# jondeaton/PhaMers

Hardware: AMD Instinct MI355X
Metric: Gbases/s k-mer-count+score, k=4, 5 kb contigs (higher is better)
Workload: dtype u32 counts + f16 MFMA proposal (exact integer counts x fp16 reference parts, f32 accumulate; k=4: high parts in the sweep, low parts added in f64 to the window's candidates) + f64 decision; 1 GPU; BASELINE configs[1]: k=4, 1000000 x 5000-base contigs per GPU, count+normalise+combo score, 4510 reference rows + 172 centroids; contigs_per_gpu=1000000, contig_length=5000, k=4, method=combo, parallelism=contig shards, 1 rank(s), replicated reference, final all-gather of scores

## Files before the change

### phamers_amd/csrc/phk_common.h

```cpp
#pragma once
#include <hip/hip_runtime.h>
#include <stdint.h>
#include <stdarg.h>
#include <stdio.h>
#include <string>
#include <thread>
#include <functional>
#include <vector>

#include "../../include/phamers_hip.h"

#define PHK_WAVE 64

#if (defined(I8_TIMERS) || defined(I8_NW) || defined(I8_NBUF) || defined(PHK_HI_REFINE) || \
     defined(PHK_RERANK_WAVES) || defined(PAIRS_ABL) || defined(F16H_ABL)) && !defined(PHK_DIAGNOSTIC_BUILD)
#error "kernel tuning / timer macros need -DPHK_DIAGNOSTIC_BUILD (make EXTRA_CXXFLAGS='-DPHK_DIAGNOSTIC_BUILD -D...')"
#endif

void phk_set_error(const char *fmt, ...);

#define PHK_HIP(call)                                                                      \
    do {                                                                                   \
        hipError_t e__ = (call);                                                           \
        if (e__ != hipSuccess) {                                                           \
            phk_set_error("%s failed: %s (%s:%d)", #call, hipGetErrorString(e__), __FILE__, \
                          __LINE__);                                                       \
            return e__ == hipErrorOutOfMemory ? PHK_ERR_NOMEM : PHK_ERR_HIP;               \
        }                                                                                  \
    } while (0)

#define PHK_REQUIRE(cond, ...)        \
    do {                              \
        if (!(cond)) {                \
            phk_set_error(__VA_ARGS__); \
            return PHK_ERR_ARG;       \
        }                             \
    } while (0)

#define PHK_ENTER(ctx_, fname)                                   \
    do {                                                         \
        PHK_REQUIRE((ctx_) != nullptr, fname ": NULL ctx");      \
        PHK_HIP(hipSetDevice((ctx_)->device));                   \
    } while (0)

#define PHK_TRY(call)               \
    do {                            \
        int rc__ = (call);          \
        if (rc__ != PHK_OK) return rc__; \
    } while (0)

enum PhkSlot {
    WS_ASCII = 0,
    WS_PACKED,
    WS_MASK,
    WS_OFFSETS,
    WS_COUNTS,
    WS_WIDE,
    WS_FLAGS,
    WS_Q64,
    WS_SCORES,
    WS_DIST,
    WS_QF32,
    WS_CAND,
    WS_NWIN,
    WS_LONG,
    WS_OUT,
    WS_SUB,
    WS_QUEUE,
    WS_FRAG8,
    WS_BIG8,
    WS_SCTL,
    WS_CTL,
    WS_KDE,
    WS_SORT,
    WS_NN,
    WS_NNF,
    WS_NND,
    WS_SLOTS
};

struct PhkBuf {
    void *ptr = nullptr;
    uint64_t bytes = 0;
    uint64_t gen = 0;
};

struct PhkTimed {
    std::string name;
    std::vector<hipEvent_t> ev;
    double ms = 0.0;
    uint64_t launches = 0;
};

struct PhkLayout {
    uint64_t bytes = 0;
    uint64_t align = 256;
    uint64_t take(uint64_t b) {
        const uint64_t o = bytes;
        bytes += (b + align - 1) / align * align;
        return o;
    }
};

enum PhkProposal { PHK_PROP_DEFAULT = 0, PHK_PROP_OTHER, PHK_PROP_F16, PHK_PROP_HI, PHK_PROP_CXF, PHK_PROP_I83 };

struct PhkKnobs {
    char count_lanes = 0;
    bool force_exact = false;
    PhkProposal proposal = PHK_PROP_DEFAULT;
    char cx_cfg[8] = "";
    char rerank = 0;
    bool count_sort = true;
    uint64_t score_batch = 0;
    char i8_insert = 0;
    bool gen_seq = false;
    int gen_groups = 0;
    int ws_fail = 0;
    bool tail_aside = true;
};

#define PHK_PREP8_MISSING 0x40000000u
#define PHK_I8_L1_MAX 65000u
struct PhkPrep8 {
    bool offered = false;
    bool written = false;
    const uint32_t *counts = nullptr;
    uint64_t n = 0, D = 0;
    void *frag = nullptr;
    uint32_t *big = nullptr;
};

struct PhkStepLink {
    PhkPrep8 prep8;
    uint32_t *zero[2] = {nullptr, nullptr};
    uint32_t zero_words[2] = {0, 0};
    bool planned = false;
    bool zeroed(const uint32_t *p) const { return planned && p && (p == zero[0] || p == zero[1]); }
};

struct phk_ctx {
    int device = 0;
    PhkKnobs knobs;
    bool slots_lds0 = true;
    hipStream_t stream = nullptr;
    bool own_stream = false;
    hipStream_t aux = nullptr;
    hipEvent_t ev_fork[2] = {nullptr, nullptr}, ev_tail[2] = {nullptr, nullptr};
    uint64_t ctl_gen = 0, ctl_epoch = 0;
    bool ctl_dirty = true;
    uint64_t score_ctl_gen = 0;
    bool score_ctl_dirty = true;
    int num_cus = 256;
    PhkBuf ws[WS_SLOTS];
    bool profile = false;
    bool last_score_fast = false;
    std::vector<PhkTimed> timed;
    std::vector<hipEvent_t> ev_pool;
    void *stage[2] = {nullptr, nullptr};
    uint64_t stage_bytes = 0;
    uint64_t nn_queries = 0, nn_fell_back = 0;
    bool nn_keep = false;
    uint64_t nn_det_n = 0;
    int nn_det_k = 0;
};

int phk_ws(phk_ctx *ctx, int slot, uint64_t bytes, void **out);

struct phk_batch {
// ... 112 lines not shown
```

### phamers_amd/csrc/score_decide.hip

```cpp
#include "score_decide.h"

template <int SRC>
__global__ __launch_bounds__(256) void phk_decide_kernel(const void *__restrict__ src, RerankParams p) {
    __shared__ uint32_t s_ix[2][256];
    __shared__ double s_T[256], s_nq2[256], s_nqp2[256], s_dp2[256], s_dn2[256], s_opQ[256], s_opI[256], s_opH[256];
    const int tid = threadIdx.x, lane = tid & 63, t = lane & 15;
    const int QB = blockDim.x;
    const uint64_t qb = (uint64_t)blockIdx.x * QB;
    const bool want_knn = (p.method & PHK_METHOD_KNN) != 0, want_cen = (p.method & PHK_METHOD_KMEANS) != 0;

    auto rowptr = [&](int pass) {
        const int ql = pass * (QB / 16) + (tid >> 4);
        const uint64_t q = qb + ql < p.N ? qb + ql : p.N - 1;
        return reinterpret_cast<const uint2 *>(static_cast<const uint32_t *>(src) + q * FAST_D) + t;
    };
    uint2 pre[2][8];
    if (SRC == 0) {
#pragma unroll
        for (int i = 0; i < 8; ++i) {
            pre[0][i] = rowptr(0)[16 * i];
            pre[1][i] = rowptr(1)[16 * i];
        }
    }

// ... 230 lines not shown
                const bool up = x > v[k];
                const float tv = v[k];
                const uint32_t ti = ix[k];
                v[k] = up ? x : tv;
                ix[k] = up ? xi : ti;
                x = up ? tv : x;
                xi = up ? ti : xi;
            }
        }
        gap_hi[sg] = need == 1 ? v[0] : need == 2 ? v[1] : v[2];
        gap_lo[sg] = need == 1 ? v[1] : need == 2 ? v[2] : v[3];
        filled[sg] = (need == 1 ? ix[0] : need == 2 ? ix[1] : ix[2]) < ncols;
#pragma unroll
        for (int r = 0; r < 3; ++r) lead[sg][r] = ix[r];
    }
    s_ix[0][tid] = lead[1][0] < (uint32_t)p.n_cpos ? lead[1][0] : 0u;
    s_ix[1][tid] = lead[2][0] < (uint32_t)p.n_cneg ? lead[2][0] : 0u;
    {
        uint32_t fl = 0;
#pragma unroll
        for (int sg = 0; sg < NSEG; ++sg) {
            s_gap[sg][0][tid] = gap_hi[sg];
            s_gap[sg][1][tid] = gap_lo[sg];
            s_gap[sg][2][tid] = Useg[sg];
            fl |= filled[sg] ? 1u << sg : 0u;
        }
#pragma unroll
        for (int r = 0; r < 3; ++r) fl |= p.labels[lead[0][r] < (uint32_t)p.M ? lead[0][r] : 0u] ? 16u << r : 0u;
        s_flag[tid] = fl;
    }
    __syncthreads();

#pragma unroll 1
    for (int pass = 0; pass < 16; ++pass) {
        const int ql = pass * 4 + grp;
        const uint64_t q = qb + ql < p.N ? qb + ql : p.N - 1;
        const double Tq = (double)p.rowsum[q];
        const uint4 *row = reinterpret_cast<const uint4 *>(counts + q * D) + t;
        const double *cp = p.C64 + (uint64_t)s_ix[0][ql] * D, *cn = p.C64 + (p.n_cpos + (uint64_t)s_ix[1][ql]) * D;
        double ssq = 0.0, ap = 0.0, dp[4] = {0.0, 0.0, 0.0, 0.0}, dn[4] = {0.0, 0.0, 0.0, 0.0};
#pragma unroll 1
        for (int ch = 0; ch < NCH; ++ch) {
#pragma unroll 1
            for (int io = 0; io < LPC / 4; ++io) {
            uint4 c[4];
#pragma unroll
            for (int i = 0; i < 4; ++i) c[i] = row[ch * (CHUNK / 4) + 16 * (4 * io + i)];
#pragma unroll
            for (int i = 0; i < 4; ++i) {
                const int d0 = ch * CHUNK + 64 * (4 * io + i) + 4 * t;
                const double x[4] = {(double)c[i].x, (double)c[i].y, (double)c[i].z, (double)c[i].w};
                const double2 m0 = *reinterpret_cast<const double2 *>(s_mu + d0), m1 = *reinterpret_cast<const double2 *>(s_mu + d0 + 2);
                const double mu4[4] = {m0.x, m0.y, m1.x, m1.y};
                double2 a0 = {0.0, 0.0}, a1 = {0.0, 0.0}, b0 = {0.0, 0.0}, b1 = {0.0, 0.0};
                if (want_cen) {
                    a0 = *reinterpret_cast<const double2 *>(cp + d0); a1 = *reinterpret_cast<const double2 *>(cp + d0 + 2);
                    b0 = *reinterpret_cast<const double2 *>(cn + d0); b1 = *reinterpret_cast<const double2 *>(cn + d0 + 2);
                }
                const double ca[4] = {a0.x, a0.y, a1.x, a1.y}, cb[4] = {b0.x, b0.y, b1.x, b1.y};
#pragma unroll
                for (int e = 0; e < 4; ++e) {
                    ssq = fma(x[e], x[e], ssq);
                    const double qm = fma(-Tq, mu4[e], x[e]);
                    ap = fma(qm, qm, ap);
                }
                if (want_cen) {
                    const double e0 = fma(-Tq, ca[0], x[0]), e1 = fma(-Tq, ca[1], x[1]), e2 = fma(-Tq, ca[2], x[2]), e3 = fma(-Tq, ca[3], x[3]);
                    dp[i & 3] = fma(e0, e0, fma(e1, e1, fma(e2, e2, fma(e3, e3, dp[i & 3]))));
                    const double f0 = fma(-Tq, cb[0], x[0]), f1 = fma(-Tq, cb[1], x[1]), f2 = fma(-Tq, cb[2], x[2]), f3 = fma(-Tq, cb[3], x[3]);
                    dn[i & 3] = fma(f0, f0, fma(f1, f1, fma(f2, f2, fma(f3, f3, dn[i & 3]))));
                }
            }
            }
        }
        ssq = group16_sum(ssq);
        ap = group16_sum(ap);
        double dps = 0.0, dns = 0.0;
        if (want_cen) {
            dps = (group16_sum(dp[0]) + group16_sum(dp[1])) + (group16_sum(dp[2]) + group16_sum(dp[3]));
            dns = (group16_sum(dn[0]) + group16_sum(dn[1])) + (group16_sum(dn[2]) + group16_sum(dn[3]));
        }
        if (t == 0) {
            s_ssq[ql] = ssq;
            s_nqp2[ql] = ap;
            s_dp2[ql] = dps;
            s_dn2[ql] = dns;
        }
    }
    __syncthreads();

    bool slow = false;
    if (in_a) {
        const uint32_t Tu = p.rowsum[qa];
        const uint32_t fl = s_flag[tid];
        if (Tu == 0u) {
            p.scores[p.q_base + qa] = __builtin_nan("");
            if (p.status) atomicAdd(p.status, 1u);
        } else {
            const double Tq = (double)Tu, ry = 1.0 / Tq, invT2 = 1.0 / (Tq * Tq);
            const double ssq = s_ssq[tid], nqp2 = s_nqp2[tid] * invT2;
            const double vs = p.vscale * ry;
            const double rcen = (double)phk_row_center(Tu, D);
            const CenteredOperand cop = phk_centered_operand_fast(ssq, Tq, ry, rcen, rcen, (double)D, p.eb_hsum);
            ErrBound eb;
            eb.A = phk_sqrt_up(ssq * (ry * ry) * (1.0 + 1e-12)) + p.mu_norm;
            eb.P = phk_sqrt_up(nqp2 + cop.shift2);
            eb.Q = cop.Q; eb.I = cop.I; eb.habs = cop.habs;
            eb.cA = p.eb_cA; eb.cP = p.eb_cP; eb.cR = p.eb_cR; eb.cabs = p.eb_abs; eb.cQ = p.eb_cQ; eb.cI = p.eb_cI; eb.cIf = p.eb_cIf;
            const double eps_g = eb(p.rmax);
            auto as_it_stands = [&](int sg) {
                if (!((fl >> sg) & 1u)) return false;
                const double el = cop.Q * p.lam8[sg] * (1.0 + 1.0e-6);
                const double thr = (double)s_gap[sg][0][tid] * vs - 2.0 * (el + eps_g);
                return (double)s_gap[sg][2][tid] * vs < thr && (double)s_gap[sg][1][tid] * vs < thr;
            };
            bool ok = true;
            double knn = 0.0;
            if (want_knn) {
                ok = as_it_stands(0);
                int votes = 0;
                for (int r = 0; r < p.kn; ++r) votes += (fl >> (4 + r)) & 1u;
                knn = (2 * votes > p.kn) ? 1.0 : -1.0;
            }
            if (want_cen) ok = ok && as_it_stands(1) && as_it_stands(2);
            if (ok) {
                if (want_cen) {
                    const uint64_t oq = p.out_map ? (uint64_t)p.out_map[qa] : qa;
                    if (p.pend) {
                        p.pend[2 * oq] = s_dp2[tid] * invT2;
                        p.pend[2 * oq + 1] = s_dn2[tid] * invT2;
                        p.scores[p.q_base + oq] = knn;
                    } else {
                        const double ep = sqrt(s_dp2[tid] * invT2), en = sqrt(s_dn2[tid] * invT2);
                        p.scores[p.q_base + oq] = knn + tanh((en - ep) / (ep + en));
                    }
                } else {
                    p.scores[p.q_base + (p.out_map ? (uint64_t)p.out_map[qa] : qa)] = knn;
                }
            } else {
                slow = true;
            }
        }
    }
    const unsigned long long sm = __ballot(slow);
    if (sm) {
        uint32_t base = 0;
        if (tid == 0) base = atomicAdd(p.fb_count + 2, (uint32_t)__popcll(sm));
        base = __shfl(base, 0);
        if (slow) p.slow_list[base + (uint32_t)__popcll(sm & ((1ull << tid) - 1ull))] = (uint32_t)qa;
    }
}

template <bool KNN, bool CEN>
__global__ __launch_bounds__(64) void phk_decide_h_kernel(const uint32_t *__restrict__ counts, RerankParams p, HiParams hp) {
    __shared__ uint32_t s_c0[8][64];
    __shared__ uint32_t s_ix[2][64];
    __shared__ float s_corr[PHK_HI_REFINE][64];
    __shared__ float s_v8[8][64], s_u0[64], s_ch[4][64];
    __shared__ double s_cn[5][64];
    __shared__ uint32_t s_flags[64];
    __shared__ double s_T[64], s_sumsq[64], s_apsum[64], s_dp2[64], s_dn2[64];
    __shared__ uint32_t s_cmx[64], s_cmn[64];
    __shared__ double s_mu[FAST_D];
    const int tid = threadIdx.x, t = tid & 15;
    const uint64_t qb = (uint64_t)blockIdx.x * 64;
    constexpr bool want_knn = KNN, want_cen = CEN;
    auto rowptr = [&](int pass) {
        const int ql = pass * 4 + (tid >> 4);
        const uint64_t q = qb + ql < p.N ? qb + ql : p.N - 1;
        return reinterpret_cast<const uint2 *>(counts + q * FAST_D) + t;
    };
    uint2 cur[8];
#pragma unroll
    for (int i = 0; i < 8; ++i) cur[i] = rowptr(0)[16 * i];
    {
        const double2 m2a = reinterpret_cast<const double2 *>(p.mu64)[2 * tid], m2b = reinterpret_cast<const double2 *>(p.mu64)[2 * tid + 1];
        reinterpret_cast<double2 *>(s_mu)[2 * tid] = m2a;
        reinterpret_cast<double2 *>(s_mu)[2 * tid + 1] = m2b;
    }

    const uint64_t qa = qb + tid;
    const bool in_a = qa < p.N;
    const uint64_t qc = in_a ? qa : p.N - 1;
    float v8[8];
    uint32_t i8[8];
    float U0 = 0.f;
    bool ok0 = true;
    float ch1[2] = {0.f, 0.f}, ch2[2] = {0.f, 0.f};
    uint32_t cl[2] = {0u, 0u};
    bool cfill[2] = {true, true};
    {
        float lv[NSEG][8], lu[2] = {0.f, 0.f};
        uint32_t li[NSEG][8];
        if (KNN) {
            lu[0] = p.cand_u[candu_at(0, 0, qc, p.N)];
            lu[1] = p.cand_u[candu_at(0, 1, qc, p.N)];
        }
#pragma unroll
        for (int sg = 0; sg < NSEG; ++sg)
            if (sg == 0 ? KNN : CEN) {
#pragma unroll
                for (int c = 0; c < 8; ++c) {
                    li[sg][c] = p.cand_i[cand_at(sg, c >> 2, c & 3, qc, p.N)];
                    lv[sg][c] = p.cand_v[cand_at(sg, c >> 2, c & 3, qc, p.N)];
                }
            }
        __builtin_amdgcn_sched_barrier(0);
        if (KNN) {
            U0 = fmaxf(lu[0], lu[1]);
#pragma unroll
            for (int c = 0; c < 8; ++c) {
                v8[c] = li[0][c] >= (uint32_t)p.M ? -3.0e38f : lv[0][c];
                i8[c] = li[0][c];
            }
#pragma unroll
            for (int a = 1; a < 8; ++a)
#pragma unroll
                for (int b = a; b > 0; --b) {
                    const bool sw = v8[b] > v8[b - 1];
                    const float tv = v8[b]; const uint32_t ti = i8[b];
                    v8[b] = sw ? v8[b - 1] : v8[b]; i8[b] = sw ? i8[b - 1] : i8[b];
                    v8[b - 1] = sw ? tv : v8[b - 1]; i8[b - 1] = sw ? ti : i8[b - 1];
                }
        }
        if (CEN) {
#pragma unroll
            for (int sg = 1; sg <= 2; ++sg) {
                const uint32_t ncols = sg == 1 ? (uint32_t)p.n_cpos : (uint32_t)p.n_cneg;
                float b1 = -3.0e38f, b2 = -3.0e38f;
                uint32_t bi = 0xFFFFFFFFu;
#pragma unroll
                for (int c = 0; c < 8; ++c) {
                    const uint32_t ix = li[sg][c];
                    const float w = ix >= ncols ? -3.0e38f : lv[sg][c];
                    const bool up = w > b1;
                    b2 = up ? b1 : fmaxf(b2, w);
                    bi = up ? ix : bi;
                    b1 = up ? w : b1;
                }
                ch1[sg - 1] = b1; ch2[sg - 1] = b2; cl[sg - 1] = bi;
                cfill[sg - 1] = bi < ncols;
            }
        }
    }
    const uint32_t ixp = cl[0] < (uint32_t)p.n_cpos ? cl[0] : 0u, ixn = cl[1] < (uint32_t)p.n_cneg ? cl[1] : 0u;
    s_ix[0][tid] = ixp;
    s_ix[1][tid] = ixn;
    {
        double cn0[3];
        uint8_t lab[8];
        uint32_t c8[8];
#pragma unroll
        for (int r = 0; r < 8; ++r) c8[r] = (KNN && i8[r] < (uint32_t)p.M) ? i8[r] : 0u;
#pragma unroll
        for (int r = 0; r < 8; ++r) {
            if (r < 3) cn0[r] = p.colnorm[c8[r]];
            lab[r] = p.labels[c8[r]];
        }
        const double cnp = p.colnorm[p.M + ixp], cnn = p.colnorm[p.M + p.n_cpos + ixn];
        __builtin_amdgcn_sched_barrier(0);
        uint32_t labbits = 0;
#pragma unroll
        for (int r = 0; r < 8; ++r) {
            labbits |= (uint32_t)(lab[r] ? 1u : 0u) << r;
            s_c0[r][tid] = c8[r];
            s_v8[r][tid] = (KNN && i8[r] < (uint32_t)p.M) ? v8[r] : -3.0e38f;
        }
        if (KNN) ok0 = i8[p.kn - 1] < (uint32_t)p.M;
        s_u0[tid] = U0;
        s_ch[0][tid] = ch1[0]; s_ch[1][tid] = ch2[0]; s_ch[2][tid] = ch1[1]; s_ch[3][tid] = ch2[1];
        s_cn[0][tid] = cn0[0]; s_cn[1][tid] = cn0[1]; s_cn[2][tid] = cn0[2]; s_cn[3][tid] = cnp; s_cn[4][tid] = cnn;
        s_flags[tid] = labbits | (ok0 ? 0x100u : 0u) | (cfill[0] ? 0x200u : 0u) | (cfill[1] ? 0x400u : 0u);
    }
    __syncthreads();

#pragma unroll 2
    for (int pass = 0; pass < 16; ++pass) {
        const int ql = pass * 4 + (tid >> 4);
        double2 ca[8], cb[8];
        uint4 l0[PHK_HI_REFINE], l1[PHK_HI_REFINE];
        uint2 nxt[8];
        if (CEN) {
            const double2 *ra = reinterpret_cast<const double2 *>(p.C64 + (uint64_t)s_ix[0][ql] * FAST_D) + t;
            const double2 *rb = reinterpret_cast<const double2 *>(p.C64 + (p.n_cpos + (uint64_t)s_ix[1][ql]) * FAST_D) + t;
#pragma unroll
            for (int i = 0; i < 8; ++i) {
                ca[i] = ra[16 * i];
                cb[i] = rb[16 * i];
            }
        }
        if (KNN) {
#pragma unroll
            for (int r = 0; r < PHK_HI_REFINE; ++r) {
                const uint4 *lp = reinterpret_cast<const uint4 *>(hp.lo16 + (uint64_t)s_c0[r][ql] * FAST_D) + t;
                l0[r] = lp[0];
                l1[r] = lp[16];
            }
        }
        {
            const uint2 *nrow = rowptr((pass + 1) & 15);
#pragma unroll
            for (int i = 0; i < 8; ++i) nxt[i] = nrow[16 * i];
        }
        __builtin_amdgcn_sched_barrier(0);
        double qd[16];
        uint32_t sum = 0, cmx = 0, cmn = 0xFFFFFFFFu;
#pragma unroll
        for (int i = 0; i < 8; ++i) {
            const uint2 c = cur[i];
            sum += c.x + c.y;
            cmx = max(cmx, max(c.x, c.y));
            cmn = min(cmn, min(c.x, c.y));
            qd[2 * i + 0] = (double)c.x;
            qd[2 * i + 1] = (double)c.y;
        }
        sum = group16_sum(sum);
        cmx = group16_max(cmx);
        cmn = group16_min(cmn);
        const bool bad = sum == 0;
        const double Tq = (double)sum;
        double dp2 = 0.0, dn2 = 0.0;
        if (CEN) {
            double acca = 0.0, accb = 0.0;
#pragma unroll
            for (int i = 0; i < 8; ++i) {
                const double a0 = fma(-Tq, ca[i].x, qd[2 * i]), a1 = fma(-Tq, ca[i].y, qd[2 * i + 1]);
                const double b0 = fma(-Tq, cb[i].x, qd[2 * i]), b1 = fma(-Tq, cb[i].y, qd[2 * i + 1]);
                acca = fma(a0, a0, fma(a1, a1, acca));
                accb = fma(b0, b0, fma(b1, b1, accb));
            }
            dp2 = group16_sum(acca);
            dn2 = group16_sum(accb);
        }
        double aq = 0.0, ap = 0.0;
#pragma unroll
        for (int i = 0; i < 8; ++i) {
            const double2 m2 = reinterpret_cast<const double2 *>(s_mu)[16 * i + t];
            aq = fma(qd[2 * i], qd[2 * i], fma(qd[2 * i + 1], qd[2 * i + 1], aq));
            qd[2 * i] = fma(-Tq, m2.x, qd[2 * i]);
            qd[2 * i + 1] = fma(-Tq, m2.y, qd[2 * i + 1]);
            ap = fma(qd[2 * i], qd[2 * i], fma(qd[2 * i + 1], qd[2 * i + 1], ap));
        }
        const double sumsq = group16_sum(aq), apsum = group16_sum(ap);
        if (KNN) {
            const double dlt = (double)phk_row_center(sum, FAST_D) - Tq * (1.0 / FAST_D);
            float qf[16];
#pragma unroll
            for (int i = 0; i < 16; ++i) qf[i] = (float)(qd[i] - dlt);
#pragma unroll
            for (int r = 0; r < PHK_HI_REFINE; ++r) {
                const _Float16 *lh0 = reinterpret_cast<const _Float16 *>(&l0[r]), *lh1 = reinterpret_cast<const _Float16 *>(&l1[r]);
                float acc = 0.f;
#pragma unroll
                for (int i = 0; i < 8; ++i) {
                    acc = fmaf(qf[i], (float)lh0[i], acc);
                    acc = fmaf(qf[8 + i], (float)lh1[i], acc);
                }
                acc = group16_sum(acc);
                if (t == 0) s_corr[r][ql] = acc;
            }
        }
        if (t == 0) {
            s_T[ql] = bad ? 0.0 : Tq;
            s_sumsq[ql] = sumsq;
            s_apsum[ql] = apsum;
            s_dp2[ql] = dp2;
            s_dn2[ql] = dn2;
            s_cmx[ql] = cmx;
            s_cmn[ql] = cmn;
        }
#pragma unroll
        for (int i = 0; i < 8; ++i) cur[i] = nxt[i];
    }
    __syncthreads();

    if (!in_a) return;
    const double Tq = s_T[tid];
    if (Tq == 0.0) {
        p.scores[p.q_base + qa] = __builtin_nan("");
        if (p.status) atomicAdd(p.status, 1u);
        return;
    }
    const double invT2 = 1.0 / (Tq * Tq);
    const double nq2 = s_sumsq[tid] * invT2, nqp2 = s_apsum[tid] * invT2;
    const CenteredOperand cop = phk_centered_operand(s_sumsq[tid], Tq, (double)s_cmx[tid], (double)s_cmn[tid], (double)FAST_D, p.eb_hsum);
    const double vs = p.vscale / Tq;
    double cn0[3];
    uint32_t labbits;
    {
#pragma unroll
        for (int r = 0; r < 8; ++r) v8[r] = s_v8[r][tid];
        U0 = s_u0[tid];
        ch1[0] = s_ch[0][tid]; ch2[0] = s_ch[1][tid]; ch1[1] = s_ch[2][tid]; ch2[1] = s_ch[3][tid];
        cn0[0] = s_cn[0][tid]; cn0[1] = s_cn[1][tid]; cn0[2] = s_cn[2][tid];
        const uint32_t fl = s_flags[tid];
        labbits = fl & 0xFFu;
        ok0 = (fl & 0x100u) != 0;
        cfill[0] = (fl & 0x200u) != 0;
        cfill[1] = (fl & 0x400u) != 0;
    }
    const double cnp2 = s_cn[3][tid], cnn2 = s_cn[4][tid];
    ErrBound eb;
    eb.A = sqrt(nq2) + p.mu_norm;
    eb.P = sqrt(nqp2);
    eb.Q = cop.Q; eb.I = cop.I; eb.habs = cop.habs + p.eb_babs;
    eb.cA = p.eb_cA; eb.cP = p.eb_cP; eb.cR = p.eb_cR; eb.cabs = p.eb_abs; eb.cQ = p.eb_cQ; eb.cI = p.eb_cI; eb.cIf = p.eb_cIf;
    eb.cM = p.eb_cM; eb.M = p.eb_M;
    const double nqp = eb.P;
    const double nqx = sqrt(nqp2 + cop.shift2);
    auto e_hi = [&](int sg, double R) { return nqx * phk_lam_of(hp, sg, R) + eb(R); };
    bool cert = true;
    bool cert_c = true;
    double knn = 0.0, cen = 0.0;
    if (want_knn) {
        const int need = p.kn;
        cert = ok0;
        if (cert) {
            const double eg = e_hi(0, p.rmax);
            const double d2up = fmax(nqp2 - 2.0 * ((double)v8[need - 1] * vs - eg), 0.0);
            const double R0 = fmin(p.rmax, (nqp + sqrt(d2up)) * (1.0 + 1e-6));
            bool near = true;
            for (int r = 0; r < need; ++r) near = near && cn0[r] <= R0;
            const double Rw = near ? R0 : p.rmax;
            const double eh = near ? e_hi(0, R0) : eg, e22 = eb(Rw) + 0x1p-19 * nqx * phk_lam_of(hp, 0, Rw);
            const double thr = (double)v8[need - 1] * vs - 2.0 * eh;
            int nw = 0;
#pragma unroll
            for (int r = 0; r < 8; ++r) nw += ((double)v8[r] * vs >= thr && v8[r] > -1.0e38f) ? 1 : 0;
            cert = nw <= PHK_HI_REFINE && (double)U0 * vs < thr;
            if (!cert && nw > PHK_HI_REFINE) atomicAdd(phk_stat_word(p, p.counters + 8, 8), 1u);
            if (!cert && nw <= PHK_HI_REFINE) atomicAdd(phk_stat_word(p, p.counters + 9, 9), 1u);
            if (cert) {
                double rv[PHK_HI_REFINE];
                uint32_t rl[PHK_HI_REFINE];
#pragma unroll
                for (int r = 0; r < PHK_HI_REFINE; ++r) {
                    const bool in = r < nw;
                    rv[r] = in ? ((double)v8[r] + (double)s_corr[r][tid]) * vs : -1.0e300;
                    rl[r] = (labbits >> r) & 1u;
                }
#pragma unroll
                for (int a = 1; a < PHK_HI_REFINE; ++a)
#pragma unroll
                    for (int b = a; b > 0; --b) {
                        const bool sw = rv[b] > rv[b - 1];
                        const double tv = rv[b]; const uint32_t tl = rl[b];
                        rv[b] = sw ? rv[b - 1] : rv[b]; rl[b] = sw ? rl[b - 1] : rl[b];
                        rv[b - 1] = sw ? tv : rv[b - 1]; rl[b - 1] = sw ? tl : rl[b - 1];
                    }
                const double hi_v = need == 1 ? rv[0] : need == 2 ? rv[1] : rv[2];
                const double lo_v = need == 1 ? rv[1] : need == 2 ? rv[2] : rv[3];
                cert = nw == need || hi_v - lo_v > 2.0 * e22;
                if (!cert) atomicAdd(phk_stat_word(p, p.counters + 10, 10), 1u);
                int votes = 0;
                for (int r = 0; r < need; ++r) votes += (int)rl[r];
                knn = (2 * votes > need) ? 1.0 : -1.0;
            }
        }
    }
    if (want_cen) {
        auto leader_ok = [&](int k2, double cnorm) {
            if (!cfill[k2]) return false;
            const double eg = e_hi(1 + k2, p.rmax);
            const double d2up = fmax(nqp2 - 2.0 * ((double)ch1[k2] * vs - eg), 0.0);
            const double R0 = fmin(p.rmax, (nqp + sqrt(d2up)) * (1.0 + 1e-6));
            const double eh = cnorm <= R0 ? e_hi(1 + k2, R0) : eg;
            return ((double)ch1[k2] - (double)ch2[k2]) * vs > 2.0 * eh;
        };
        cert_c = leader_ok(0, cnp2) && leader_ok(1, cnn2);
        if (!cert_c) atomicAdd(phk_stat_word(p, p.counters + 11, 11), 1u);
        const double ep = sqrt(s_dp2[tid] * invT2), en = sqrt(s_dn2[tid] * invT2);
        cen = tanh((en - ep) / (ep + en));
    }
    if (cert && cert_c) {
        p.scores[p.q_base + qa] = knn + cen;
    } else {
        p.scores[p.q_base + qa] = (cert ? knn : 0.0) + (cert_c ? cen : 0.0);
        const uint32_t open_parts = ((want_knn && !cert) ? 1u : 0u) | ((want_cen && !cert_c) ? 2u : 0u);
        if (p.sub_lists) {
            const uint32_t sl = blockIdx.x % p.sub_lists;
            uint32_t *cw = p.stripes + sl * 32u;
            const uint64_t base = (uint64_t)sl * p.sub_cap;
            if (open_parts == 2u) p.slow_list[base + p.sub_cap - 1 - atomicAdd(cw + 12, 1u)] = (uint32_t)qa | (open_parts << 30);
            else p.slow_list[base + atomicAdd(cw + 2, 1u)] = (uint32_t)qa | (open_parts << 30);
        } else if (open_parts == 2u) p.slow_list[p.slow_cap - 1 - atomicAdd(p.counters + 12, 1u)] = (uint32_t)qa | (open_parts << 30);
        else p.slow_list[atomicAdd(p.fb_count + 2, 1u)] = (uint32_t)qa | (open_parts << 30);
    }
}

int phk_launch_decide(phk_ctx *ctx, int src_kind, const void *src, const RerankParams &p) {
    const dim3 grid((unsigned)phk_div_up(p.N, 64));
    if (src_kind == 0) { PHK_LAUNCH(ctx, "phk_decide_kernel", phk_decide_kernel<0><<<grid, dim3(64), 0, ctx->stream>>>(src, p)); }
    else { PHK_LAUNCH(ctx, "phk_decide_kernel", phk_decide_kernel<1><<<grid, dim3(64), 0, ctx->stream>>>(src, p)); }
    return PHK_OK;
}

int phk_launch_decide_gen(phk_ctx *ctx, int dsub, const uint32_t *counts, const RerankParams &p) {
    const dim3 grid((unsigned)phk_div_up(p.N, 64));
#define PHK_DG(DS) PHK_LAUNCH(ctx, "phk_decide_gen_kernel", (phk_decide_gen_kernel<DS><<<grid, dim3(64), 0, ctx->stream>>>(counts, p)))
    switch (dsub) {
        case 2: PHK_DG(2); break;
        case 4: PHK_DG(4); break;
        case 8: PHK_DG(8); break;
        case 16: PHK_DG(16); break;
        default: phk_set_error("phk_launch_decide_gen: D = %d", 256 * dsub); return PHK_ERR_UNSUPPORTED;
    }
#undef PHK_DG
    return PHK_OK;
}

int phk_launch_decide_h(phk_ctx *ctx, bool knn, bool cen, dim3 grid, dim3 block, const uint32_t *counts, const RerankParams &p, const HiParams &hp) {
    PHK_REQUIRE(knn || cen, "phk_launch_decide_h: nothing to decide");
    if (knn && cen) { PHK_LAUNCH(ctx, "phk_decide_h_kernel", (phk_decide_h_kernel<true, true><<<grid, block, 0, ctx->stream>>>(counts, p, hp))); }
    else if (knn) { PHK_LAUNCH(ctx, "phk_decide_h_kernel", (phk_decide_h_kernel<true, false><<<grid, block, 0, ctx->stream>>>(counts, p, hp))); }
    else { PHK_LAUNCH(ctx, "phk_decide_h_kernel", (phk_decide_h_kernel<false, true><<<grid, block, 0, ctx->stream>>>(counts, p, hp))); }
    return PHK_OK;
}
```

Before: 1473 Gbases/s.

## Compact fp16 low-part refinement to only queries whose window has ties

The decide kernel used to load the low fp16 reference parts for every query's top candidates and compute correction dot products during the main 16-pass sweep. Now the certification bounds are evaluated first, the queries that actually need refinement (certified with more window candidates than k) are compacted into a shared list, and only those rows are reloaded and corrected in a second, wave-compacted loop. The change also keeps mu in registers instead of shared memory, shares LDS between the row sums and the correction buffer through a union, and adds an occupancy hint to the launch bounds. In exchange, refined rows are read twice, extra barriers are added, and register pressure under the new launch bound may cause spills.

```diff
diff --git a/phamers_amd/csrc/phk_common.h b/phamers_amd/csrc/phk_common.h
--- a/phamers_amd/csrc/phk_common.h
+++ b/phamers_amd/csrc/phk_common.h
@@ -13,7 +13,8 @@
 #define PHK_WAVE 64
 
 #if (defined(I8_TIMERS) || defined(I8_NW) || defined(I8_NBUF) || defined(PHK_HI_REFINE) || \
-     defined(PHK_RERANK_WAVES) || defined(PAIRS_ABL) || defined(F16H_ABL)) && !defined(PHK_DIAGNOSTIC_BUILD)
+     defined(PHK_RERANK_WAVES) || defined(PAIRS_ABL) || defined(F16H_ABL) || defined(PHK_DECIDE_H_CLASSES)) && \
+    !defined(PHK_DIAGNOSTIC_BUILD)
 #error "kernel tuning / timer macros need -DPHK_DIAGNOSTIC_BUILD (make EXTRA_CXXFLAGS='-DPHK_DIAGNOSTIC_BUILD -D...')"
 #endif
 
diff --git a/phamers_amd/csrc/score_decide.hip b/phamers_amd/csrc/score_decide.hip
--- a/phamers_amd/csrc/score_decide.hip
+++ b/phamers_amd/csrc/score_decide.hip
@@ -406,32 +406,27 @@
 }
 
 template <bool KNN, bool CEN>
-__global__ __launch_bounds__(64) void phk_decide_h_kernel(const uint32_t *__restrict__ counts, RerankParams p, HiParams hp) {
-    __shared__ uint32_t s_c0[8][64];
+__global__ __launch_bounds__(64, 3) void phk_decide_h_kernel(const uint32_t *__restrict__ counts, RerankParams p, HiParams hp) {
+    __shared__ uint32_t s_c0[PHK_HI_REFINE][64];
     __shared__ uint32_t s_ix[2][64];
-    __shared__ float s_corr[PHK_HI_REFINE][64];
     __shared__ float s_v8[8][64], s_u0[64], s_ch[4][64];
     __shared__ double s_cn[5][64];
     __shared__ uint32_t s_flags[64];
-    __shared__ double s_T[64], s_sumsq[64], s_apsum[64], s_dp2[64], s_dn2[64];
-    __shared__ uint32_t s_cmx[64], s_cmn[64];
-    __shared__ double s_mu[FAST_D];
+    __shared__ double s_T[64], s_dp2[64], s_dn2[64];
+    struct RowSums { double sumsq[64], apsum[64]; uint32_t cmx[64], cmn[64]; };
+    __shared__ union { RowSums row; float corr[PHK_HI_REFINE][64]; } s_w;
+    __shared__ uint8_t s_list[64];
     const int tid = threadIdx.x, t = tid & 15;
     const uint64_t qb = (uint64_t)blockIdx.x * 64;
     constexpr bool want_knn = KNN, want_cen = CEN;
-    auto rowptr = [&](int pass) {
-        const int ql = pass * 4 + (tid >> 4);
+    auto rowptr_of = [&](int ql) {
         const uint64_t q = qb + ql < p.N ? qb + ql : p.N - 1;
         return reinterpret_cast<const uint2 *>(counts + q * FAST_D) + t;
     };
+    auto rowptr = [&](int pass) { return rowptr_of(pass * 4 + (tid >> 4)); };
     uint2 cur[8];
 #pragma unroll
     for (int i = 0; i < 8; ++i) cur[i] = rowptr(0)[16 * i];
-    {
-        const double2 m2a = reinterpret_cast<const double2 *>(p.mu64)[2 * tid], m2b = reinterpret_cast<const double2 *>(p.mu64)[2 * tid + 1];
-        reinterpret_cast<double2 *>(s_mu)[2 * tid] = m2a;
-        reinterpret_cast<double2 *>(s_mu)[2 * tid + 1] = m2b;
-    }
 
     const uint64_t qa = qb + tid;
     const bool in_a = qa < p.N;
@@ -517,7 +512,7 @@
 #pragma unroll
         for (int r = 0; r < 8; ++r) {
             labbits |= (uint32_t)(lab[r] ? 1u : 0u) << r;
-            s_c0[r][tid] = c8[r];
+            if (r < PHK_HI_REFINE) s_c0[r][tid] = c8[r];
             s_v8[r][tid] = (KNN && i8[r] < (uint32_t)p.M) ? v8[r] : -3.0e38f;
         }
         if (KNN) ok0 = i8[p.kn - 1] < (uint32_t)p.M;
@@ -528,11 +523,14 @@
     }
     __syncthreads();
 
+    double2 mu[8];
+#pragma unroll
+    for (int i = 0; i < 8; ++i) mu[i] = reinterpret_cast<const double2 *>(p.mu64)[16 * i + t];
+
 #pragma unroll 2
     for (int pass = 0; pass < 16; ++pass) {
         const int ql = pass * 4 + (tid >> 4);
         double2 ca[8], cb[8];
-        uint4 l0[PHK_HI_REFINE], l1[PHK_HI_REFINE];
         uint2 nxt[8];
         if (CEN) {
             const double2 *ra = reinterpret_cast<const double2 *>(p.C64 + (uint64_t)s_ix[0][ql] * FAST_D) + t;
@@ -543,21 +541,12 @@
                 cb[i] = rb[16 * i];
             }
         }
-        if (KNN) {
-#pragma unroll
-            for (int r = 0; r < PHK_HI_REFINE; ++r) {
-                const uint4 *lp = reinterpret_cast<const uint4 *>(hp.lo16 + (uint64_t)s_c0[r][ql] * FAST_D) + t;
-                l0[r] = lp[0];
-                l1[r] = lp[16];
-            }
-        }
         {
             const uint2 *nrow = rowptr((pass + 1) & 15);
 #pragma unroll
             for (int i = 0; i < 8; ++i) nxt[i] = nrow[16 * i];
         }
         __builtin_amdgcn_sched_barrier(0);
-        double qd[16];
         uint32_t sum = 0, cmx = 0, cmn = 0xFFFFFFFFu;
 #pragma unroll
         for (int i = 0; i < 8; ++i) {
@@ -565,164 +554,211 @@
             sum += c.x + c.y;
             cmx = max(cmx, max(c.x, c.y));
             cmn = min(cmn, min(c.x, c.y));
-            qd[2 * i + 0] = (double)c.x;
-            qd[2 * i + 1] = (double)c.y;
         }
         sum = group16_sum(sum);
         cmx = group16_max(cmx);
         cmn = group16_min(cmn);
         const bool bad = sum == 0;
         const double Tq = (double)sum;
+        double aq = 0.0, ap = 0.0, acca = 0.0, accb = 0.0;
+#pragma unroll
+        for (int i = 0; i < 8; ++i) {
+            const double x0 = (double)cur[i].x, x1 = (double)cur[i].y;
+            if (CEN) {
+                const double a0 = fma(-Tq, ca[i].x, x0), a1 = fma(-Tq, ca[i].y, x1);
+                const double b0 = fma(-Tq, cb[i].x, x0), b1 = fma(-Tq, cb[i].y, x1);
+                acca = fma(a0, a0, fma(a1, a1, acca));
+                accb = fma(b0, b0, fma(b1, b1, accb));
+            }
+            aq = fma(x0, x0, fma(x1, x1, aq));
+            const double y0 = fma(-Tq, mu[i].x, x0), y1 = fma(-Tq, mu[i].y, x1);
+            ap = fma(y0, y0, fma(y1, y1, ap));
+        }
         double dp2 = 0.0, dn2 = 0.0;
         if (CEN) {
-            double acca = 0.0, accb = 0.0;
-#pragma unroll
-            for (int i = 0; i < 8; ++i) {
-                const double a0 = fma(-Tq, ca[i].x, qd[2 * i]), a1 = fma(-Tq, ca[i].y, qd[2 * i + 1]);
-                const double b0 = fma(-Tq, cb[i].x, qd[2 * i]), b1 = fma(-Tq, cb[i].y, qd[2 * i + 1]);
-                acca = fma(a0, a0, fma(a1, a1, acca));
-                accb = fma(b0, b0, fma(b1, b1, accb));
-            }
             dp2 = group16_sum(acca);
             dn2 = group16_sum(accb);
         }
-        double aq = 0.0, ap = 0.0;
-#pragma unroll
-        for (int i = 0; i < 8; ++i) {
-            const double2 m2 = reinterpret_cast<const double2 *>(s_mu)[16 * i + t];
-            aq = fma(qd[2 * i], qd[2 * i], fma(qd[2 * i + 1], qd[2 * i + 1], aq));
-            qd[2 * i] = fma(-Tq, m2.x, qd[2 * i]);
-            qd[2 * i + 1] = fma(-Tq, m2.y, qd[2 * i + 1]);
-            ap = fma(qd[2 * i], qd[2 * i], fma(qd[2 * i + 1], qd[2 * i + 1], ap));
-        }
         const double sumsq = group16_sum(aq), apsum = group16_sum(ap);
-        if (KNN) {
-            const double dlt = (double)phk_row_center(sum, FAST_D) - Tq * (1.0 / FAST_D);
-            float qf[16];
-#pragma unroll
-            for (int i = 0; i < 16; ++i) qf[i] = (float)(qd[i] - dlt);
-#pragma unroll
-            for (int r = 0; r < PHK_HI_REFINE; ++r) {
-                const _Float16 *lh0 = reinterpret_cast<const _Float16 *>(&l0[r]), *lh1 = reinterpret_cast<const _Float16 *>(&l1[r]);
-                float acc = 0.f;
-#pragma unroll
-                for (int i = 0; i < 8; ++i) {
-                    acc = fmaf(qf[i], (float)lh0[i], acc);
-                    acc = fmaf(qf[8 + i], (float)lh1[i], acc);
-                }
-                acc = group16_sum(acc);
-                if (t == 0) s_corr[r][ql] = acc;
-            }
-        }
         if (t == 0) {
             s_T[ql] = bad ? 0.0 : Tq;
-            s_sumsq[ql] = sumsq;
-            s_apsum[ql] = apsum;
+            s_w.row.sumsq[ql] = sumsq;
+            s_w.row.apsum[ql] = apsum;
             s_dp2[ql] = dp2;
             s_dn2[ql] = dn2;
-            s_cmx[ql] = cmx;
-            s_cmn[ql] = cmn;
+            s_w.row.cmx[ql] = cmx;
+            s_w.row.cmn[ql] = cmn;
         }
 #pragma unroll
         for (int i = 0; i < 8; ++i) cur[i] = nxt[i];
     }
     __syncthreads();
 
-    if (!in_a) return;
     const double Tq = s_T[tid];
-    if (Tq == 0.0) {
+    bool live = in_a;
+    if (live && Tq == 0.0) {
         p.scores[p.q_base + qa] = __builtin_nan("");
         if (p.status) atomicAdd(p.status, 1u);
-        return;
+        live = false;
     }
     const double invT2 = 1.0 / (Tq * Tq);
-    const double nq2 = s_sumsq[tid] * invT2, nqp2 = s_apsum[tid] * invT2;
-    const CenteredOperand cop = phk_centered_operand(s_sumsq[tid], Tq, (double)s_cmx[tid], (double)s_cmn[tid], (double)FAST_D, p.eb_hsum);
     const double vs = p.vscale / Tq;
-    double cn0[3];
-    uint32_t labbits;
-    {
-#pragma unroll
-        for (int r = 0; r < 8; ++r) v8[r] = s_v8[r][tid];
-        U0 = s_u0[tid];
-        ch1[0] = s_ch[0][tid]; ch2[0] = s_ch[1][tid]; ch1[1] = s_ch[2][tid]; ch2[1] = s_ch[3][tid];
-        cn0[0] = s_cn[0][tid]; cn0[1] = s_cn[1][tid]; cn0[2] = s_cn[2][tid];
-        const uint32_t fl = s_flags[tid];
-        labbits = fl & 0xFFu;
-        ok0 = (fl & 0x100u) != 0;
-        cfill[0] = (fl & 0x200u) != 0;
-        cfill[1] = (fl & 0x400u) != 0;
-    }
-    const double cnp2 = s_cn[3][tid], cnn2 = s_cn[4][tid];
-    ErrBound eb;
-    eb.A = sqrt(nq2) + p.mu_norm;
-    eb.P = sqrt(nqp2);
-    eb.Q = cop.Q; eb.I = cop.I; eb.habs = cop.habs + p.eb_babs;
-    eb.cA = p.eb_cA; eb.cP = p.eb_cP; eb.cR = p.eb_cR; eb.cabs = p.eb_abs; eb.cQ = p.eb_cQ; eb.cI = p.eb_cI; eb.cIf = p.eb_cIf;
-    eb.cM = p.eb_cM; eb.M = p.eb_M;
-    const double nqp = eb.P;
-    const double nqx = sqrt(nqp2 + cop.shift2);
-    auto e_hi = [&](int sg, double R) { return nqx * phk_lam_of(hp, sg, R) + eb(R); };
+    const uint32_t fl = s_flags[tid];
     bool cert = true;
     bool cert_c = true;
+    int nw = 0;
+    bool refine = false;
+    double e22 = 0.0;
+    {
+        const double nq2 = s_w.row.sumsq[tid] * invT2, nqp2 = s_w.row.apsum[tid] * invT2;
+        const CenteredOperand cop = phk_centered_operand(s_w.row.sumsq[tid], Tq, (double)s_w.row.cmx[tid], (double)s_w.row.cmn[tid], (double)FAST_D, p.eb_hsum);
+        ErrBound eb;
+        eb.A = sqrt(nq2) + p.mu_norm;
+        eb.P = sqrt(nqp2);
+        eb.Q = cop.Q; eb.I = cop.I; eb.habs = cop.habs + p.eb_babs;
+        eb.cA = p.eb_cA; eb.cP = p.eb_cP; eb.cR = p.eb_cR; eb.cabs = p.eb_abs; eb.cQ = p.eb_cQ; eb.cI = p.eb_cI; eb.cIf = p.eb_cIf;
+        eb.cM = p.eb_cM; eb.M = p.eb_M;
+        const double nqp = eb.P;
+        const double nqx = sqrt(nqp2 + cop.shift2);
+        auto e_hi = [&](int sg, double R) { return nqx * phk_lam_of(hp, sg, R) + eb(R); };
+        if (want_knn) {
+            const int need = p.kn;
+#pragma unroll
+            for (int r = 0; r < 8; ++r) v8[r] = s_v8[r][tid];
+            U0 = s_u0[tid];
+            const double cn0[3] = {s_cn[0][tid], s_cn[1][tid], s_cn[2][tid]};
+            cert = live && (fl & 0x100u) != 0;
+            if (cert) {
+                const double eg = e_hi(0, p.rmax);
+                const double d2up = fmax(nqp2 - 2.0 * ((double)v8[need - 1] * vs - eg), 0.0);
+                const double R0 = fmin(p.rmax, (nqp + sqrt(d2up)) * (1.0 + 1e-6));
+                bool near = true;
+                for (int r = 0; r < need; ++r) near = near && cn0[r] <= R0;
+                const double Rw = near ? R0 : p.rmax;
+                const double eh = near ? e_hi(0, R0) : eg;
+                e22 = eb(Rw) + 0x1p-19 * nqx * phk_lam_of(hp, 0, Rw);
+                const double thr = (double)v8[need - 1] * vs - 2.0 * eh;
+#pragma unroll
+                for (int r = 0; r < 8; ++r) nw += ((double)v8[r] * vs >= thr && v8[r] > -1.0e38f) ? 1 : 0;
+                cert = nw <= PHK_HI_REFINE && (double)U0 * vs < thr;
+#if defined(PHK_DIAGNOSTIC_BUILD) && defined(PHK_DECIDE_H_CLASSES)
+                if (cert && nw == need) atomicAdd(phk_stat_word(p, p.counters + 8, 8), 1u);
+                if (cert && nw != need) atomicAdd(phk_stat_word(p, p.counters + 9, 9), 1u);
+                if (cert && nw != need) atomicAdd(phk_stat_word(p, p.counters + 10, 10), (uint32_t)nw);
+#else
+                if (!cert && nw > PHK_HI_REFINE) atomicAdd(phk_stat_word(p, p.counters + 8, 8), 1u);
+                if (!cert && nw <= PHK_HI_REFINE) atomicAdd(phk_stat_word(p, p.counters + 9, 9), 1u);
+#endif
+                refine = cert && nw != need;
+                s_flags[tid] = fl | ((uint32_t)nw << 12);
+            }
+        }
+        if (want_cen) {
+            ch1[0] = s_ch[0][tid]; ch2[0] = s_ch[1][tid]; ch1[1] = s_ch[2][tid]; ch2[1] = s_ch[3][tid];
+            cfill[0] = (fl & 0x200u) != 0;
+            cfill[1] = (fl & 0x400u) != 0;
+            const double cnp2 = s_cn[3][tid], cnn2 = s_cn[4][tid];
+            auto leader_ok = [&](int k2, double cnorm) {
+                if (!cfill[k2]) return false;
+                const double eg = e_hi(1 + k2, p.rmax);
+                const double d2up = fmax(nqp2 - 2.0 * ((double)ch1[k2] * vs - eg), 0.0);
+                const double R0 = fmin(p.rmax, (nqp + sqrt(d2up)) * (1.0 + 1e-6));
+                const double eh = cnorm <= R0 ? e_hi(1 + k2, R0) : eg;
+                return ((double)ch1[k2] - (double)ch2[k2]) * vs > 2.0 * eh;
+            };
+            cert_c = leader_ok(0, cnp2) && leader_ok(1, cnn2);
+            if (live && !cert_c) atomicAdd(phk_stat_word(p, p.counters + 11, 11), 1u);
+        }
+    }
+
+    if (KNN) {
+        const unsigned long long rmask = __ballot(refine);
+        __syncthreads();
+        if (rmask) {
+            if (refine) s_list[__popcll(rmask & ((1ull << tid) - 1ull))] = (uint8_t)tid;
+            __syncthreads();
+            const int nref = __popcll(rmask);
+            double2 mu2[8];
+#pragma unroll
+            for (int i = 0; i < 8; ++i) mu2[i] = reinterpret_cast<const double2 *>(p.mu64)[16 * i + t];
+#pragma unroll 1
+            for (int base = 0; base < nref; base += 4) {
+                const int e = base + (tid >> 4);
+                const int ql = s_list[e < nref ? e : nref - 1];
+                const int nwq = e < nref ? (int)((s_flags[ql] >> 12) & 15u) : 0;
+                const double Tr = s_T[ql];
+                uint2 row[8];
+                uint4 l0[PHK_HI_REFINE], l1[PHK_HI_REFINE];
+                {
+                    const uint2 *rp = rowptr_of(ql);
+#pragma unroll
+                    for (int i = 0; i < 8; ++i) row[i] = rp[16 * i];
+                }
+#pragma unroll
+                for (int r = 0; r < PHK_HI_REFINE; ++r) {
+                    const uint4 *lp = reinterpret_cast<const uint4 *>(hp.lo16 + (uint64_t)s_c0[r < nwq ? r : 0][ql] * FAST_D) + t;
+                    l0[r] = lp[0];
+                    l1[r] = lp[16];
+                }
+                __builtin_amdgcn_sched_barrier(0);
+                const double dlt = (double)phk_row_center((uint32_t)Tr, FAST_D) - Tr * (1.0 / FAST_D);
+                float qf[16];
+#pragma unroll
+                for (int i = 0; i < 8; ++i) {
+                    qf[2 * i] = (float)(fma(-Tr, mu2[i].x, (double)row[i].x) - dlt);
+                    qf[2 * i + 1] = (float)(fma(-Tr, mu2[i].y, (double)row[i].y) - dlt);
+                }
+#pragma unroll
+                for (int r = 0; r < PHK_HI_REFINE; ++r)
+                    if (__ballot(r < nwq)) {
+                        const _Float16 *lh0 = reinterpret_cast<const _Float16 *>(&l0[r]), *lh1 = reinterpret_cast<const _Float16 *>(&l1[r]);
+                        float acc = 0.f;
+#pragma unroll
+                        for (int i = 0; i < 8; ++i) {
+                            acc = fmaf(qf[i], (float)lh0[i], acc);
+                            acc = fmaf(qf[8 + i], (float)lh1[i], acc);
+                        }
+                        acc = group16_sum(acc);
+                        if (t == 0 && r < nwq) s_w.corr[r][ql] = acc;
+                    }
+            }
+            __syncthreads();
+        }
+    }
+
+    if (!live) return;
     double knn = 0.0, cen = 0.0;
-    if (want_knn) {
+    if (want_knn && cert) {
         const int need = p.kn;
-        cert = ok0;
-        if (cert) {
-            const double eg = e_hi(0, p.rmax);
-            const double d2up = fmax(nqp2 - 2.0 * ((double)v8[need - 1] * vs - eg), 0.0);
-            const double R0 = fmin(p.rmax, (nqp + sqrt(d2up)) * (1.0 + 1e-6));
-            bool near = true;
-            for (int r = 0; r < need; ++r) near = near && cn0[r] <= R0;
-            const double Rw = near ? R0 : p.rmax;
-            const double eh = near ? e_hi(0, R0) : eg, e22 = eb(Rw) + 0x1p-19 * nqx * phk_lam_of(hp, 0, Rw);
-            const double thr = (double)v8[need - 1] * vs - 2.0 * eh;
-            int nw = 0;
-#pragma unroll
-            for (int r = 0; r < 8; ++r) nw += ((double)v8[r] * vs >= thr && v8[r] > -1.0e38f) ? 1 : 0;
-            cert = nw <= PHK_HI_REFINE && (double)U0 * vs < thr;
-            if (!cert && nw > PHK_HI_REFINE) atomicAdd(phk_stat_word(p, p.counters + 8, 8), 1u);
-            if (!cert && nw <= PHK_HI_REFINE) atomicAdd(phk_stat_word(p, p.counters + 9, 9), 1u);
-            if (cert) {
-                double rv[PHK_HI_REFINE];
-                uint32_t rl[PHK_HI_REFINE];
-#pragma unroll
-                for (int r = 0; r < PHK_HI_REFINE; ++r) {
-                    const bool in = r < nw;
-                    rv[r] = in ? ((double)v8[r] + (double)s_corr[r][tid]) * vs : -1.0e300;
-                    rl[r] = (labbits >> r) & 1u;
-                }
-#pragma unroll
-                for (int a = 1; a < PHK_HI_REFINE; ++a)
-#pragma unroll
-                    for (int b = a; b > 0; --b) {
-                        const bool sw = rv[b] > rv[b - 1];
-                        const double tv = rv[b]; const uint32_t tl = rl[b];
-                        rv[b] = sw ? rv[b - 1] : rv[b]; rl[b] = sw ? rl[b - 1] : rl[b];
-                        rv[b - 1] = sw ? tv : rv[b - 1]; rl[b - 1] = sw ? tl : rl[b - 1];
-                    }
-                const double hi_v = need == 1 ? rv[0] : need == 2 ? rv[1] : rv[2];
-                const double lo_v = need == 1 ? rv[1] : need == 2 ? rv[2] : rv[3];
-                cert = nw == need || hi_v - lo_v > 2.0 * e22;
-                if (!cert) atomicAdd(phk_stat_word(p, p.counters + 10, 10), 1u);
-                int votes = 0;
-                for (int r = 0; r < need; ++r) votes += (int)rl[r];
-                knn = (2 * votes > need) ? 1.0 : -1.0;
-            }
-        }
+        double rv[PHK_HI_REFINE];
+        uint32_t rl[PHK_HI_REFINE];
+#pragma unroll
+        for (int r = 0; r < PHK_HI_REFINE; ++r) {
+            const bool in = r < nw;
+            const float corr = (in && refine) ? s_w.corr[r][tid] : 0.f;
+            rv[r] = in ? ((double)s_v8[r][tid] + (double)corr) * vs : -1.0e300;
+            rl[r] = (fl >> r) & 1u;
+        }
+#pragma unroll
+        for (int a = 1; a < PHK_HI_REFINE; ++a)
+#pragma unroll
+            for (int b = a; b > 0; --b) {
+                const bool sw = rv[b] > rv[b - 1];
+                const double tv = rv[b]; const uint32_t tl = rl[b];
+                rv[b] = sw ? rv[b - 1] : rv[b]; rl[b] = sw ? rl[b - 1] : rl[b];
+                rv[b - 1] = sw ? tv : rv[b - 1]; rl[b - 1] = sw ? tl : rl[b - 1];
+            }
+        const double hi_v = need == 1 ? rv[0] : need == 2 ? rv[1] : rv[2];
+        const double lo_v = need == 1 ? rv[1] : need == 2 ? rv[2] : rv[3];
+        cert = nw == need || hi_v - lo_v > 2.0 * e22;
+#if !(defined(PHK_DIAGNOSTIC_BUILD) && defined(PHK_DECIDE_H_CLASSES))
+        if (!cert) atomicAdd(phk_stat_word(p, p.counters + 10, 10), 1u);
+#endif
+        int votes = 0;
+        for (int r = 0; r < need; ++r) votes += (int)rl[r];
+        knn = (2 * votes > need) ? 1.0 : -1.0;
     }
     if (want_cen) {
-        auto leader_ok = [&](int k2, double cnorm) {
-            if (!cfill[k2]) return false;
-            const double eg = e_hi(1 + k2, p.rmax);
-            const double d2up = fmax(nqp2 - 2.0 * ((double)ch1[k2] * vs - eg), 0.0);
-            const double R0 = fmin(p.rmax, (nqp + sqrt(d2up)) * (1.0 + 1e-6));
-            const double eh = cnorm <= R0 ? e_hi(1 + k2, R0) : eg;
-            return ((double)ch1[k2] - (double)ch2[k2]) * vs > 2.0 * eh;
-        };
-        cert_c = leader_ok(0, cnp2) && leader_ok(1, cnn2);
-        if (!cert_c) atomicAdd(phk_stat_word(p, p.counters + 11, 11), 1u);
         const double ep = sqrt(s_dp2[tid] * invT2), en = sqrt(s_dn2[tid] * invT2);
         cen = tanh((en - ep) / (ep + en));
     }
```

After: 1483 Gbases/s (median of 4 runs). No clear change (+0.6%).
